# hinike/cairo

Measured on AMD Instinct MI355X. Metric: encoded Mpixels/s (p-frame, q=16) at 1/2/4/8 MI355X; bit-exact vs ref, higher is better.
Workload: dtype int16

## Files before the change

cairo_amd/__init__.py:

```python
from __future__ import annotations

import ctypes
import os
from dataclasses import dataclass

import numpy as np

_HERE = os.path.dirname(os.path.abspath(__file__))
LIB_PATH = os.path.join(_HERE, "_lib", "libcairo_amd.so")

BLOCK_DESC = np.dtype(
    [
        ("block_type", "<u4"),
        ("prediction_target", "u1"),
        ("pad", "u1"),
        ("motion_x", "<i2"),
        ("motion_y", "<i2"),
        ("sp_pred", "u1"),
        ("sp_amount", "u1"),
        ("sp_index", "u1"),
        ("q_index", "u1"),
        ("variance", "<i2"),
    ]
)
# ... 87 lines not shown
        "cairo_stream_payload_bits": (I, [P, I, ctypes.POINTER(ctypes.c_uint64)]),
        "cairo_bits_append": (I, [P, ctypes.c_uint64, ctypes.POINTER(ctypes.c_uint64), P, ctypes.c_uint64]),
        "evx_encoder_create": (I, [ctypes.POINTER(P)]),
        "evx_encoder_destroy": (I, [P]),
        "evx_encoder_clear": (I, [P]),
        "evx_encoder_insert_intra": (I, [P]),
        "evx_encoder_set_quality": (I, [P, ctypes.c_uint8]),
        "evx_encoder_encode": (I, [P, P, U, U, P]),
        "evx_encoder_set_ring": (I, [P, U]),
        "evx_encoder_peek": (I, [P, I, P]),
        "evx_encoder_set_device": (I, [P, I]),
        "evx_bitstream_create": (P, [U]),
        "evx_bitstream_destroy": (V, [P]),
        "evx_bitstream_data": (P, [P]),
        "evx_bitstream_occupancy": (U, [P]),
        "evx_bitstream_empty": (V, [P]),
        "evx_bitstream_write_bits": (I, [P, P, U]),
        "evx_decoder_create": (I, [ctypes.POINTER(P)]),
        "evx_decoder_destroy": (I, [P]),
        "evx_decoder_clear": (I, [P]),
        "evx_decoder_decode": (I, [P, P, P]),
        "evx_decoder_set_device": (I, [P, I]),
        "cairo_ctx_decode_frame": (I, [P, P, P, U, P]),
        "cairo_make_band4": (V, [P, U, U, U, U]),
        "cairo_version": (ctypes.c_char_p, []),
        "cairo_api_version": (I, []),
        "cairo_device_count": (I, []),
    }
    for name, (res, args) in sig.items():
        fn = getattr(L, name)
        fn.restype = res
        fn.argtypes = args
    if L.cairo_api_version() != API_VERSION:
        raise ImportError(f"{LIB_PATH} has C ABI version {L.cairo_api_version()}, these bindings expect "
                          f"{API_VERSION} (include/cairo_amd.h CAIRO_AMD_API_VERSION): rebuild with `make`")
    _lib = L
    return L


def _ck(status: int, what: str) -> None:
    if status != EVX_SUCCESS:
        raise CairoError(what, status)


def _ptr(a: np.ndarray) -> int:
    assert a.flags["C_CONTIGUOUS"]
    return a.ctypes.data


def _host_frame(rgb, width: int, height: int) -> int:
    if not isinstance(rgb, np.ndarray):
        raise TypeError("host frames are numpy arrays (pass on_device=True for a device address)")
    if rgb.dtype != np.uint8 or rgb.shape != (height, width, 3) or not rgb.flags["C_CONTIGUOUS"]:
        raise ValueError(f"frame must be a C-contiguous uint8 array of shape ({height}, {width}, 3), "
                         f"got {rgb.dtype} {rgb.shape}")
    return rgb.ctypes.data


def make_band4(w: int, h: int, t: int, seed: int = 1234) -> np.ndarray:
    out = np.empty((h, w, 3), np.uint8)
    lib().cairo_make_band4(_ptr(out), w, h, t, seed)
    return out


class _FrameResult(ctypes.Structure):
    _fields_ = [
        ("block_table", ctypes.c_void_p),
        ("coef_y", ctypes.c_void_p),
        ("coef_u", ctypes.c_void_p),
        ("coef_v", ctypes.c_void_p),
        ("wa", ctypes.c_uint32),
        ("ha", ctypes.c_uint32),
        ("wmb", ctypes.c_uint32),
        ("hmb", ctypes.c_uint32),
        ("index", ctypes.c_uint32),
        ("type", ctypes.c_uint32),
        ("quality", ctypes.c_uint32),
        ("feed", ctypes.c_void_p),
        ("feed_bits", ctypes.c_uint64),
        ("feed_status", ctypes.c_int32),
    ]


@dataclass
class FrameOutputs:

    table: np.ndarray
    coef_y: np.ndarray | None
    coef_u: np.ndarray | None
    coef_v: np.ndarray | None
    feed: np.ndarray | None = None
    feed_bits: int = 0
    feed_status: int = 0


def _view(addr: int, dtype, count: int) -> np.ndarray:
    buf = (ctypes.c_char * (count * np.dtype(dtype).itemsize)).from_address(addr)
    return np.frombuffer(buf, dtype=dtype, count=count)


class Context:

    def __init__(self, width: int, height: int, ring: int = 4, device: int = 0, stages: int = 96):
        self.L = lib()
        self.width, self.height, self.ring, self.device = width, height, ring, device
        self.wa, self.ha = (width + 15) & ~15, (height + 15) & ~15
        self.wmb, self.hmb = self.wa // 16, self.ha // 16
        p = ctypes.c_void_p()
        _ck(self.L.cairo_ctx_create_ex(width, height, ring, device, stages, ctypes.byref(p)), "cairo_ctx_create")
        self.h = p
        self._keep = {}

    def close(self) -> None:
        if self.h:
            self.L.cairo_ctx_destroy(self.h)
            self.h = None

    def __del__(self):
        try:
            self.close()
        except Exception:
            pass

    @property
    def stages(self) -> int:
        return int(self.L.cairo_ctx_stages(self.h))

    def submit(self, rgb, index: int, inter: bool, quality: int, on_device: bool = False) -> int:
        t = ctypes.c_int()
        ptr = rgb if on_device else _host_frame(rgb, self.width, self.height)
        _ck(
            self.L.cairo_ctx_submit(self.h, ptr, int(on_device), index, int(inter), quality, ctypes.byref(t)),
            "cairo_ctx_submit",
        )
        if not on_device:
            self._keep[t.value] = rgb
        return t.value

    def wait(self, ticket: int, copy: bool = True) -> FrameOutputs:
        r = _FrameResult()
        st = self.L.cairo_ctx_wait(self.h, ticket, ctypes.byref(r))
        if st != EVX_SUCCESS:
            raise CairoError("cairo_ctx_wait", st, self.timeout_info() if st == EVX_ERROR_HARDWAREFAIL else None)
        self._keep.pop(ticket, None)
        return self._outputs(r, copy)

    ACCT_FIELDS = ("coder_tasks", "coder_total", "coder_group_wait", "coder_window", "coder_search", "coder_inter",
                   "coder_dequeue", "coder_mbs", "helper_tasks", "helper_total", "helper_wait", "helper_deblock",
                   "helper_search", "helper_catchup", "helper_dequeue", "helper_chunks",
                   "win_bytes", "win_spec_unused_bytes", "zero_mv_bytes", "gran_poll_bytes", "rec_poll_bytes",
                   "win_stages", "searched_tasks", "inter_tasks", "coder_xform", "coder_publish", "coder_drain",
                   "coder_vm0", "coder_records", "coder_prebarrier", "coder_store_tail",
                   "search_eval", "search_barrier", "search_select", "subpel_eval", "subpel_barrier",
                   "subpel_select", "db_inputs", "db_filter", "db_write")

    def read_acct(self, reset: bool = False) -> dict:
        w = np.zeros(len(self.ACCT_FIELDS), np.uint64)
        _ck(self.L.cairo_ctx_read_acct(self.h, _ptr(w), len(w), int(reset)), "cairo_ctx_read_acct")
        return {k: int(w[i]) for i, k in enumerate(self.ACCT_FIELDS)}

    def timeout_info(self) -> dict | None:
        w = np.zeros(16, np.int32)
        _ck(self.L.cairo_ctx_timeout_info(self.h, _ptr(w), 16), "cairo_ctx_timeout_info")
        if not w[0]:
            return None
        d = {k: int(w[i]) for i, k in enumerate(TIMEOUT_FIELDS)}
        d["kind"] = WAIT_KINDS.get(d["kind"], str(d["kind"]))
        d["seen"] = (d.pop("seen_hi") & 0xFFFFFFFF) << 32 | (d.pop("seen_lo") & 0xFFFFFFFF)
        return d

    def _outputs(self, r, copy: bool) -> FrameOutputs:
        ny, nc = r.wa * r.ha, (r.wa // 2) * (r.ha // 2)
        mbs = r.wmb * r.hmb
        has_coef = bool(r.coef_y)
        feed = _view(r.feed, np.uint32, (r.feed_bits + 31) // 32) if r.feed_status == FEED_VALID else None
        out = FrameOutputs(
            _view(r.block_table, BLOCK_DESC, mbs),
            _view(r.coef_y, np.int16, ny).reshape(r.ha, r.wa) if has_coef else None,
            _view(r.coef_u, np.int16, nc).reshape(r.ha // 2, r.wa // 2) if has_coef else None,
            _view(r.coef_v, np.int16, nc).reshape(r.ha // 2, r.wa // 2) if has_coef else None,
            feed, int(r.feed_bits), int(r.feed_status),
        )
        if copy:
            cp = lambda a: None if a is None else a.copy()
            out = FrameOutputs(cp(out.table), cp(out.coef_y), cp(out.coef_u), cp(out.coef_v), cp(out.feed),
                               out.feed_bits, out.feed_status)
        return out

    def set_outputs(self, outputs: int) -> None:
        _ck(self.L.cairo_ctx_set_outputs(self.h, outputs), "cairo_ctx_set_outputs")

    def fetch_coef(self, ticket: int):
        r = _FrameResult()
        _ck(self.L.cairo_ctx_fetch_coef(self.h, ticket, ctypes.byref(r)), "cairo_ctx_fetch_coef")
        ny, nc = self.wa * self.ha, (self.wa // 2) * (self.ha // 2)
        return (_view(r.coef_y, np.int16, ny).reshape(self.ha, self.wa).copy(),
                _view(r.coef_u, np.int16, nc).reshape(self.ha // 2, self.wa // 2).copy(),
                _view(r.coef_v, np.int16, nc).reshape(self.ha // 2, self.wa // 2).copy())

    def release(self, ticket: int) -> None:
        _ck(self.L.cairo_ctx_release(self.h, ticket), "cairo_ctx_release")

    def encode_frame(self, rgb, index: int, inter: bool, quality: int, on_device: bool = False) -> FrameOutputs:
        t = self.submit(rgb, index, inter, quality, on_device)
        try:
            return self.wait(t, copy=True)
        finally:
            self.release(t)

    def sync(self) -> None:
        _ck(self.L.cairo_ctx_sync(self.h), "cairo_ctx_sync")

    def reset(self) -> None:
        _ck(self.L.cairo_ctx_reset(self.h), "cairo_ctx_reset")
        self._keep.clear()

    def read_planes(self, which: int):
        y = np.empty((self.ha, self.wa), np.int16)
        u = np.empty((self.ha // 2, self.wa // 2), np.int16)
        v = np.empty_like(u)
        _ck(self.L.cairo_ctx_read_planes(self.h, which, _ptr(y), _ptr(u), _ptr(v)), "read_planes")
        return y, u, v

    def read_inter(self):
        n = self.wmb * self.hmb * max(self.ring - 1, 0)
        d = np.zeros(n, BLOCK_DESC)
        s = np.zeros(n, np.int32)
        if n:
            _ck(self.L.cairo_ctx_read_inter(self.h, _ptr(d), _ptr(s)), "read_inter")
        return d, s

    def read_table(self):
        t = np.zeros(self.wmb * self.hmb, BLOCK_DESC)
        _ck(self.L.cairo_ctx_read_table(self.h, _ptr(t)), "read_table")
        return t

    def set_debug(self, flags: int) -> None:
        _ck(self.L.cairo_ctx_set_debug(self.h, flags), "set_debug")

    def read_predeblock(self):
        y = np.empty((self.ha, self.wa), np.int16)
        u = np.empty((self.ha // 2, self.wa // 2), np.int16)
        v = np.empty_like(u)
        _ck(self.L.cairo_ctx_read_predeblock(self.h, _ptr(y), _ptr(u), _ptr(v)), "read_predeblock")
        return y, u, v

    def read_stamps(self):
        n_mb, n_db = self.hmb * self.wmb * 12, self.hmb * 256
        fw = n_mb + n_db
        ng = (self.wmb + 3) // 4
        n_it = MAX_BATCH * self.hmb * ng * 12
        out = np.zeros(MAX_BATCH * fw + 2 + n_it, np.uint64)
        _ck(self.L.cairo_ctx_read_stamps(self.h, _ptr(out)), "read_stamps")
        fr = out[: MAX_BATCH * fw].reshape(MAX_BATCH, fw)
        return (fr[:, :n_mb].reshape(MAX_BATCH, self.hmb, self.wmb, 12), fr[:, n_mb:].reshape(MAX_BATCH, self.hmb, 256),
                out[MAX_BATCH * fw:MAX_BATCH * fw + 2], out[MAX_BATCH * fw + 2:].reshape(MAX_BATCH, self.hmb, ng, 12))

    def set_profiling(self, enable: bool) -> None:
        _ck(self.L.cairo_ctx_set_profiling(self.h, int(enable)), "set_profiling")

    def take_timings(self):
        ms = (ctypes.c_double * 4)()
        n = ctypes.c_int()
        _ck(self.L.cairo_ctx_take_timings(self.h, ms, ctypes.byref(n)), "take_timings")
        return list(ms), n.value

    def busy_intervals(self) -> np.ndarray:
        n = ctypes.c_int()
        _ck(self.L.cairo_ctx_busy_intervals(self.h, None, 0, ctypes.byref(n)), "busy_intervals")
        out = np.zeros((max(n.value, 1), 2), np.float64)
        _ck(self.L.cairo_ctx_busy_intervals(self.h, _ptr(out), n.value, ctypes.byref(n)), "busy_intervals")
        return out[: n.value]

    def set_batch(self, frames: int) -> None:
        _ck(self.L.cairo_ctx_set_batch(self.h, frames), "set_batch")

    def set_workgroups(self, rows: int = 0) -> None:
        _ck(self.L.cairo_ctx_set_workgroups(self.h, rows), "set_workgroups")

    def set_helpers(self, helpers: int = 0) -> None:
        _ck(self.L.cairo_ctx_set_helpers(self.h, helpers), "set_helpers")

    def max_workgroups(self) -> int:
        return int(self.L.cairo_ctx_max_workgroups(self.h))

    def flush(self) -> None:
        _ck(self.L.cairo_ctx_flush(self.h), "cairo_ctx_flush")

    def peer_info(self, cross_device: bool = False) -> bytes:
        rec = (ctypes.c_uint8 * PEER_SIZE)()
        _ck(self.L.cairo_ctx_peer_info(self.h, int(cross_device), rec), "cairo_ctx_peer_info")
        return bytes(rec)

    def join_group(self, rank: int, peers: list) -> None:
        buf = b"".join(peers)
        assert len(buf) == PEER_SIZE * len(peers)
        arr = (ctypes.c_uint8 * len(buf)).from_buffer_copy(buf)
        _ck(self.L.cairo_ctx_join_group(self.h, len(peers), rank, arr), "cairo_ctx_join_group")


MIRROR_SLOTS = 16


def group_layout(n: int, size: int, ring: int, stages: int, mirror: bool = False) -> dict:
    slots = -(-ring // size)
    t = n // size
    slot = (n % size) * slots + t % slots if mirror else t % slots
# ... 323 lines not shown
```

cairo_amd/csrc/kernels.h:

```cpp
#pragma once

#include <hip/hip_runtime.h>
#include <stdint.h>

#include "evx_defs.h"

namespace cairo {

struct PlaneSet {
  int16_t* y;
  int16_t* u;
  int16_t* v;
};

__host__ __device__ inline PlaneSet ring_slot(int16_t* base, size_t slot_elems, int wa, int ha,
                                              int k) {
  PlaneSet p;
  p.y = base + (size_t)k * slot_elems;
  p.u = p.y + (size_t)wa * ha;
  p.v = p.u + (size_t)(wa / 2) * (ha / 2);
  return p;
}

constexpr int kGranulesPerMB = 192;
constexpr int kGranuleStride = 193;

__host__ __device__ inline uint32_t pack_inter_desc(const BlockDesc& d) {
  return (d.block_type & 7u) | ((uint32_t)(d.prediction_target & 3) << 3) | ((uint32_t)(d.sp_pred & 1) << 5) |
         ((uint32_t)(d.sp_amount & 1) << 6) | ((uint32_t)(d.sp_index & 15) << 7) |
         (((uint32_t)d.motion_x & 0x7Fu) << 11) | (((uint32_t)d.motion_y & 0x7Fu) << 18);
}
__host__ __device__ inline BlockDesc unpack_inter_desc(uint32_t w) {
  BlockDesc d;
  d.block_type = w & 7u;
  d.prediction_target = (uint8_t)((w >> 3) & 3);
  d.pad = 0;
  d.sp_pred = (uint8_t)((w >> 5) & 1);
  d.sp_amount = (uint8_t)((w >> 6) & 1);
  d.sp_index = (uint8_t)((w >> 7) & 15);
  d.motion_x = (int16_t)((int32_t)(w << 14) >> 25);
  d.motion_y = (int16_t)((int32_t)(w << 7) >> 25);
  d.q_index = 0;
  d.variance = 0;
  return d;
}

constexpr int kStampPhases = 12;
constexpr int kDbStamps = 256;
constexpr int kIStamps = 12;
__host__ __device__ inline size_t stamp_frame_words(int wmb, int hmb) {
  return (size_t)wmb * hmb * kStampPhases + (size_t)hmb * kDbStamps;
}

struct TimeoutInfo {
  static constexpr int kKind = 0;
  static constexpr int kEpoch = 1;
  static constexpr int kIndex = 2;
  static constexpr int kRow = 3;
  static constexpr int kMember = 4;
  static constexpr int kNeed = 5;
  static constexpr int kOn = 6;
  static constexpr int kSeenLo = 7;
  static constexpr int kSeenHi = 8;
  static constexpr int kClaim = 9;
  static constexpr int kWords = 16;
};
enum TimeoutKind : int32_t {
  kWaitRecords = 1,
  kWaitGranule = 2,
  kWaitPrevProgress = 3,
  kWaitRowAbove = 4,
  kWaitBatch = 5,
  kWaitInjected = 6,
  kWaitHostMark = 9,
};

#ifndef CAIRO_ACCT
#define CAIRO_ACCT 0
#endif
constexpr int kAcctShards = 64, kAcctWords = 40;
struct Acct {
  static constexpr int kCoderTasks = 0, kCoderTotal = 1, kCoderGroupWait = 2, kCoderWindow = 3, kCoderSearch = 4,
                       kCoderInter = 5, kCoderDequeue = 6, kCoderMBs = 7;
  static constexpr int kHelperTasks = 8, kHelperTotal = 9, kHelperWait = 10, kHelperDeblock = 11, kHelperSearch = 12,
                       kHelperCatchup = 13, kHelperDequeue = 14, kHelperChunks = 15;
  static constexpr int kWinBytes = 16, kWinSpecUnused = 17, kZeroMvBytes = 18, kGranPollBytes = 19,
                       kRecPollBytes = 20, kWinStages = 21, kSearchedTasks = 22, kInterTasks = 23;
  static constexpr int kCoderXform = 24, kCoderPublish = 25, kCoderDrain = 26;
  static constexpr int kCoderVm0 = 27, kCoderRecords = 28, kCoderPreBarrier = 29;
  static constexpr int kCoderStoreTail = 30;
  static constexpr int kSrchEval = 31, kSrchBarrier = 32, kSrchSelect = 33, kSubEval = 34, kSubBarrier = 35,
                       kSubSelect = 36;
  static constexpr int kDbInputs = 37, kDbFilter = 38, kDbWrite = 39;
};

#ifndef CAIRO_MAX_BATCH
#define CAIRO_MAX_BATCH 48
#endif
constexpr int kMaxBatch = CAIRO_MAX_BATCH;
constexpr int kMaxGroup = 16;
constexpr int kMaxPush = kMaxRing;

struct FrameDesc {
  const uint8_t* rgb;
  const uint8_t* host_rgb;
  int index;
  int inter;
  int quality;
  uint32_t epoch;
  int slot;
  int decode;
  PlaneSet recon[kMaxRing];
  PlaneSet stale;
  PlaneSet coef;
  PlaneSet push[kMaxPush];
  int npush;
  PlaneSet coef_prev;
  uint64_t* progress;
  const uint64_t* prev_progress;
  const uint64_t* prev2_progress;
  int sys;
  int member;
  const BlockDesc* host_table;
  const int16_t* host_coef;
};

struct FrameArgs {
  int wa, ha;
  int w, h;
  int wmb, hmb;
  int ring;
  int index, inter, quality;
  int decode;
  uint32_t epoch;
  PlaneSet in;
  PlaneSet coef;
  PlaneSet coef_prev;
  PlaneSet recon[kMaxRing];
  PlaneSet stale;
  PlaneSet push[kMaxPush];
  int npush;
  BlockDesc* table;
  BlockDesc* inter_desc;
  void* reserved0;
  uint64_t* granules;
  int32_t* err;
  int32_t* sticky;
  int member;
  int inject;
  int ng;
  int nref;
  int32_t* inter_done;
  uint64_t* progress;
  const uint64_t* prev_progress;
  const uint64_t* prev2_progress;
  int sys;
  int db_shift;
  uint64_t* stamps;
  uint64_t* acct;
  uint64_t* istamps;
  const uint8_t* rgb;
};

struct EngineArgs;
FrameArgs make_frame_view(const EngineArgs& e, const FrameDesc& f, int j);

struct SyncLayout {
  static constexpr int kErr = 0;
  static constexpr int kDone = 4;
  static constexpr int kLabelOff = 5;
  static constexpr int kTicketRows = 8;
  static constexpr int kTicketHelpers = 16;
  static constexpr int kFlags = 24;
  __host__ __device__ static int frame_words(int hmb, int ng) { return hmb * ng; }
  __host__ __device__ static int inter_done(int hmb, int ng, int j) { return kFlags + frame_words(hmb, ng) * j; }
  __host__ __device__ static int words(int hmb, int ng) { return kFlags + frame_words(hmb, ng) * kMaxBatch + 8; }
};

struct EngineArgs {
  int wa, ha, w, h, wmb, hmb, ring;
  int nframes;
  const FrameArgs* fa;
  int16_t* src_base;
  size_t plane_elems;
  BlockDesc* table_base;
  BlockDesc* idesc_base;
  void* reserved0;
  uint64_t* gran_base;
  int32_t* sync;
  int32_t* sticky;
  int inject;
  uint64_t* stamps;
  uint64_t* acct;
  int n_helpers, n_rows;
  int32_t* trace;
  const int32_t* order[2];
  const int32_t* seg[2];
  int nlab[2];
  int decode;
  const FrameArgs* pfa;
  const int32_t* porder[2];
  const int32_t* pseg[2];
  int32_t* psync;
  int ptotal;
  int slope;
};

constexpr int kOrderSlope = 5;

constexpr int kPrioFrameMBs = 4000;

constexpr int kLabels = 8;
constexpr int kBandMinRows = 100;
constexpr int kBandPools = 3;
__host__ __device__ inline int task_label(int frame, int row, int hmb) {
  (void)frame;
  return row * kLabels / hmb;
}

struct ConvertArgs {
  int w, h, wa, nframes;
  const uint8_t* rgb[kMaxBatch];
  PlaneSet in[kMaxBatch];
  const uint4* fa_host;
  uint4* fa_dev;
  int fa_chunks;
  int32_t* sync;
  int sync_words;
};
hipError_t launch_convert_batch(const ConvertArgs& c, hipStream_t s);
hipError_t launch_engine(const EngineArgs& e, hipStream_t s);
hipError_t launch_batch_wait(int32_t* sync, int tasks, int32_t* sticky, hipStream_t s);
hipError_t engine_blocks_per_cu(int* n);
hipError_t launch_unpack_granules(const EngineArgs& e, int j, PlaneSet dst, hipStream_t s);

hipError_t launch_yuv_to_rgb(PlaneSet src, int wa, int w, int h, uint8_t* rgb, hipStream_t s);

hipError_t launch_kat_transform(const int16_t* src, const int16_t* pred, int16_t* coef,
                                int16_t* recon, const uint8_t* qtype, int32_t* qvar,
                                int count, hipStream_t s);

}
```

cairo_amd/csrc/kernels.hip:

```cpp
#include "kernels.h"

namespace cairo {

typedef const __attribute__((address_space(4))) FrameArgs FA;
#define RECON_AT(a, k)                                                                   \
  ((k) == 1 ? planes((a).recon[1]) : (k) == 2 ? planes((a).recon[2]) : (k) == 3 ? planes((a).recon[3]) \
                                                                              : planes((a).recon[0]))
__host__ __device__ inline PlaneSet planes(const __attribute__((address_space(4))) PlaneSet& p) {
  PlaneSet r;
  r.y = p.y;
  r.u = p.u;
  r.v = p.v;
  return r;
}


__constant__ int16_t kLut8[64] = {
    128, 128,  128,  128,  128,  128,  128,  128,
    126, 106,  71,   25,   -25,  -71,  -106, -126,
    118, 49,   -49,  -118, -118, -49,  49,   118,
    106, -25,  -126, -71,  71,   126,  25,   -106,
    91,  -91,  -91,  91,   91,   -91,  -91,  91,
    71,  -126, 25,   106,  -106, -25,  126,  -71,
    49,  -118, 118,  -49,  -49,  118,  -118, 49,
// ... 399 lines not shown
  const int16_t* py = &p.y[(size_t)(y + (l >> 2)) * wa + x + (l & 3) * 4];
  int cw = wa >> 1;
  Px6 r;
  r.y0 = py[0];
  r.y1 = py[1];
  r.y2 = py[2];
  r.y3 = py[3];
  r.u = p.u[(size_t)((y >> 1) + (l >> 3)) * cw + (x >> 1) + (l & 7)];
  r.v = p.v[(size_t)((y >> 1) + (l >> 3)) * cw + (x >> 1) + (l & 7)];
  return r;
}

__device__ __forceinline__ int lerp_px(int a, int b, int quarter) {
  return quarter ? (int16_t)(round_out(3 * a + b, 2) / 4) : (int16_t)(round_out(a + b, 1) / 2);
}
__device__ __forceinline__ uint32_t lerp_half_bb(uint32_t a, uint32_t b) {
  const uint32_t t = a + b;
  return (t + ((t >> 16) & 1)) >> 1;
}
__device__ __forceinline__ uint32_t lerp_quarter_bb3(uint32_t a3, uint32_t b) {
  const uint32_t t = a3 + b;
  return (t + 1 + ((t >> 17) & 1)) >> 2;
}
__device__ __forceinline__ uint32_t lerp_quarter_bb(uint32_t a, uint32_t b) { return lerp_quarter_bb3(3 * a, b); }
__device__ __forceinline__ uint32_t absdiff_b(uint32_t x, uint32_t y) {
  return __builtin_amdgcn_sad_u16(x, y, 0);
}

__device__ __forceinline__ void inter_cand_row(const Window& w, int wx, int wy, int i, const SrcRow& s, int thr,
                                               int& sad, int& mad) {
  const int sh = (wx & 1) * 2;
  const uint32_t* row = (const uint32_t*)&w.y[(wy + i) * kWinLP] + (wx >> 1);
  uint32_t d[9];
#pragma unroll
  for (int k = 0; k < 9; k++) d[k] = row[k];
  uint32_t sm = 0;
#pragma unroll
  for (int k = 0; k < 8; k++) sm = __builtin_amdgcn_sad_u16(s.y[k], __builtin_amdgcn_alignbyte(d[k + 1], d[k], sh), sm);
  sad = row16_sum((int)sm);
  mad = kMadFar;
  if (__ballot(mad_needed(sad, thr))) {
    u16x2 m1 = {0, 0}, m2 = {0, 0};
    uint32_t dummy = 0;
#pragma unroll
    for (int k = 0; k < 8; k++) pk_diff(s.y[k], __builtin_amdgcn_alignbyte(d[k + 1], d[k], sh), dummy, m1, m2);
    const int cr = (wy >> 1) + (i >> 1), cc = (wx >> 1) + (i & 1) * 4, shc = (cc & 1) * 2;
    const uint32_t* ru = (const uint32_t*)&w.u[cr * kWinCP] + (cc >> 1);
    const uint32_t* rv = (const uint32_t*)&w.v[cr * kWinCP] + (cc >> 1);
    const uint32_t u0 = ru[0], u1 = ru[1], u2 = ru[2], v0 = rv[0], v1 = rv[1], v2 = rv[2];
    pk_diff(s.u[0], __builtin_amdgcn_alignbyte(u1, u0, shc), dummy, m1, m2);
    pk_diff(s.u[1], __builtin_amdgcn_alignbyte(u2, u1, shc), dummy, m1, m2);
    pk_diff(s.v[0], __builtin_amdgcn_alignbyte(v1, v0, shc), dummy, m1, m2);
    pk_diff(s.v[1], __builtin_amdgcn_alignbyte(v2, v1, shc), dummy, m1, m2);
    const u16x2 m = __builtin_elementwise_max(m1, m2);
    mad = row16_max(max((int)m.x, (int)m.y));
  }
}

__device__ __forceinline__ SrcRow load_src_rows(const PlaneSet& in, int wa, int px, int py, int i) {
  SrcRow s;
  const uint4* ry = (const uint4*)(in.y + (size_t)(py + i) * wa + px);
  const uint4 r0 = ry[0], r1 = ry[1];
  s.y[0] = r0.x, s.y[1] = r0.y, s.y[2] = r0.z, s.y[3] = r0.w;
  s.y[4] = r1.x, s.y[5] = r1.y, s.y[6] = r1.z, s.y[7] = r1.w;
  const size_t co = (size_t)((py >> 1) + (i >> 1)) * (wa >> 1) + (px >> 1) + (i & 1) * 4;
  const uint2 u2 = *(const uint2*)(in.u + co), v2 = *(const uint2*)(in.v + co);
  s.u[0] = u2.x, s.u[1] = u2.y, s.v[0] = v2.x, s.v[1] = v2.y;
#pragma unroll
  for (int k = 0; k < 8; k++) s.y[k] ^= 0x80008000u;
#pragma unroll
  for (int k = 0; k < 2; k++) s.u[k] ^= 0x80008000u, s.v[k] ^= 0x80008000u;
  return s;
}

__device__ __forceinline__ void sad_mad(const Px6& s, const Px6& c, int& sad, int& mad) {
  int d0 = abs(s.y0 - c.y0), d1 = abs(s.y1 - c.y1), d2 = abs(s.y2 - c.y2), d3 = abs(s.y3 - c.y3);
  int du = abs(s.u - c.u), dv = abs(s.v - c.v);
  sad = wave_sum(d0 + d1 + d2 + d3);
  mad = wave_max(max(max(max(d0, d1), max(d2, d3)), max(du, dv)));
}

struct Sel {
  int bx, by, sad, mad, ssd, sp_idx, sp_amt, sp_en;
};

__device__ __forceinline__ void accept_int(Sel& s, int cx, int cy, int sad, int mad, int px, int py,
                                           int thr) {
  int ssd = (cx - px) * (cx - px) + (cy - py) * (cy - py);
  bool acc = (s.mad < thr) ? (mad < s.mad || (mad == s.mad && ssd < s.ssd))
                           : (sad < s.sad || (sad == s.sad && ssd < s.ssd && sad < kSadGate) ||
                              mad < thr);
  if (acc) {
    s.bx = cx;
    s.by = cy;
    s.sad = sad;
    s.ssd = ssd;
    s.mad = mad;
  }
}
__device__ __forceinline__ void accept_sub(Sel& s, int idx, int quarter, int sad, int mad,
                                           int thr) {
  bool acc = (s.mad < thr) ? (mad < s.mad) : ((sad < s.sad && sad < kSadGate) || mad < thr);
  if (acc) {
    s.sp_en = 1;
    s.sp_amt = quarter;
    s.sp_idx = idx;
    s.sad = sad;
    s.mad = mad;
  }
}



__device__ __forceinline__ uint32_t row0_min(uint32_t v) {
  v = min(v, (uint32_t)__builtin_amdgcn_mov_dpp((int)v, 0x128, 0xF, 0xF, false));
  v = min(v, (uint32_t)__builtin_amdgcn_mov_dpp((int)v, 0x124, 0xF, 0xF, false));
  v = min(v, (uint32_t)__builtin_amdgcn_mov_dpp((int)v, 0x122, 0xF, 0xF, false));
  v = min(v, (uint32_t)__builtin_amdgcn_mov_dpp((int)v, 0x121, 0xF, 0xF, false));
  return (uint32_t)__builtin_amdgcn_readlane((int)v, 0);
}

__device__ __forceinline__ uint32_t key_copy(int mad, int ssd, int idx) {
  return ((uint32_t)min(mad, 65535) << 16) | ((uint32_t)min(ssd, 4095) << 4) | (uint32_t)idx;
}
__device__ __forceinline__ uint32_t key_sad(int sad, int ssd, int idx) {
  if (sad < kSadGate)
    return ((uint32_t)sad << 18) | ((uint32_t)min(ssd, 16383) << 4) | (uint32_t)idx;
  return 0x80000000u | ((uint32_t)min(sad, (1 << 27) - 1) << 4) | (uint32_t)idx;
}

__device__ __forceinline__ void select_int(Sel& s, bool valid, int cx, int cy, int sad, int mad,
                                           int px, int py, int thr, int lane) {
  const int c = lane & 15;
  const bool live = lane < 16 && valid;
  const int ssd = (cx - px) * (cx - px) + (cy - py) * (cy - py);
  const uint32_t fm = (uint32_t)__ballot(live && mad < thr);
  int w = -1;
  if (s.mad < thr || fm) {
    const int f = s.mad < thr ? -1 : (int)__builtin_ctz(fm);
    const uint32_t k = row0_min(live && c >= f ? key_copy(mad, ssd, c + 1) : 0xFFFFFFFFu);
    if (f >= 0) w = (int)(k & 15) - 1;
    else if (k < key_copy(s.mad, s.ssd, 0)) w = (int)(k & 15) - 1;
  } else {
    const uint32_t k = row0_min(live ? key_sad(sad, ssd, c + 1) : 0xFFFFFFFFu);
    if (k < key_sad(s.sad, s.ssd, 0)) w = (int)(k & 15) - 1;
  }
  if (w >= 0) {
    s.bx = __builtin_amdgcn_readlane(cx, w);
    s.by = __builtin_amdgcn_readlane(cy, w);
    s.sad = __builtin_amdgcn_readlane(sad, w);
    s.ssd = __builtin_amdgcn_readlane(ssd, w);
    s.mad = __builtin_amdgcn_readlane(mad, w);
  }
}

__device__ __forceinline__ void select_sub(Sel& s, bool valid, int sad, int mad, int thr, int lane) {
  const int c = lane & 15;
  const bool live = lane < 16 && valid;
  const uint32_t fm = (uint32_t)__ballot(live && mad < thr);
  int w = -1;
  if (s.mad < thr || fm) {
    const int f = s.mad < thr ? -1 : (int)__builtin_ctz(fm);
    const uint32_t k = row0_min(live && c >= f ? (((uint32_t)min(mad, 65535) << 5) | (uint32_t)(c + 1))
                                               : 0xFFFFFFFFu);
    if (f >= 0) w = (int)(k & 31) - 1;
    else if (k < ((uint32_t)min(s.mad, 65535) << 5)) w = (int)(k & 31) - 1;
  } else {
    const uint32_t k =
        row0_min(live && sad < kSadGate ? (((uint32_t)sad << 5) | (uint32_t)(c + 1)) : 0xFFFFFFFFu);
    if (k < ((uint32_t)min(s.sad, 1 << 26) << 5)) w = (int)(k & 31) - 1;
  }
  if (w >= 0) {
    const int n = w >> 1, k9 = n < 4 ? n : n + 1;
    s.sp_en = 1;
    s.sp_amt = w & 1;
    s.sp_idx = frac_index(k9 % 3 - 1, k9 / 3 - 1);
    s.sad = __builtin_amdgcn_readlane(sad, w);
    s.mad = __builtin_amdgcn_readlane(mad, w);
  }
}

__device__ __forceinline__ bool in_frame(int x, int y, int wa, int ha) {
  return x >= 0 && x <= wa - kMB && y >= 0 && y <= ha - kMB;
}

__device__ __forceinline__ BlockDesc make_desc(const Sel& s, int px, int py, int thr, bool intra,
                                               int target) {
  BlockDesc d;
  uint32_t t = intra ? kIntra : 0u;
  if (s.bx != px || s.by != py || s.sp_en) t |= kMotion;
  if (s.mad < thr) t |= kCopy;
  d.block_type = t;
  d.prediction_target = (uint8_t)target;
  d.pad = 0;
  d.motion_x = (int16_t)(s.bx - px);
  d.motion_y = (int16_t)(s.by - py);
  d.sp_pred = (uint8_t)s.sp_en;
  d.sp_amount = (uint8_t)s.sp_amt;
  d.sp_index = (uint8_t)s.sp_idx;
  d.q_index = 0;
  d.variance = 0;
  return d;
}


constexpr int kLvl1Rows = 77, kLvl1Cols = 112;

__device__ __forceinline__ int wg_broadcast(volatile int* slot, int v) {
  if (threadIdx.x == 0) *slot = v;
  __syncthreads();
  const int r = *slot;
  __syncthreads();
  return r;
}

struct DbLds;
struct DbState;
__device__ __forceinline__ bool deblock_chunk_ready(FA& a, int r, const DbState& st);
__device__ __forceinline__ void deblock_chunk(FA& a, int r, DbLds& D, DbState& st, bool known_ready = false);
__device__ __forceinline__ bool deblock_pending(FA& a, const DbState& st);

template <bool kDeblock = true>
__device__ __forceinline__ void helper_wait(FA& a, int back, int r, int rr, int need, DbLds& D, DbState& st,
                                            int* flag) {
  volatile int* vflag = flag;
  const uint64_t* pp = back == 1 ? a.prev_progress : a.prev2_progress;
  uint64_t t0 = 0;
  const uint64_t ta = acct_now();
  uint64_t tdb = 0;
  for (;;) {
    int d = 0;
    if (threadIdx.x == 0) {
      const uint64_t pv = pp ? progress_peer(a.sys, pp + rr) : ~0ull;
      const bool dbr = kDeblock && deblock_pending(a, st) && deblock_chunk_ready(a, r, st);
      if (a.inject && r == min(1, a.hmb - 1)) {
        report_timeout(a, kWaitInjected, r, need, rr | (back << 16), pv);
        d = 1;
      } else if (pv >= tagged(a.epoch - back, need)) {
        d = 1;
      } else if (dbr) {
        d = 2;
      } else {
        const uint64_t now = __builtin_amdgcn_s_memrealtime();
        if (!t0) t0 = now;
        __builtin_amdgcn_s_sleep(1);
        if (__hip_atomic_load(a.err, __ATOMIC_RELAXED, __HIP_MEMORY_SCOPE_AGENT)) {
          d = 1;
        } else if (now - t0 > 200000000ull) {
          report_timeout(a, kWaitPrevProgress, r, need, rr | (back << 16), pv);
          d = 1;
        }
      }
    }
    d = wg_broadcast(vflag, d);
    if (d == 1) break;
    if (kDeblock && d == 2) {
      const uint64_t tb = acct_now();
      deblock_chunk(a, r, D, st, true);
      tdb += acct_now() - tb;
    }
  }
  if (threadIdx.x == 0) {
    acquire_fence(a.sys);
    asm volatile("s_waitcnt vmcnt(0)" ::: "memory");
  }
  __syncthreads();
  acct_add(a.acct, Acct::kHelperWait, acct_now() - ta - tdb);
}

struct InterLds {
  Window win;
  int need[4];
  int full;
  int lvl2[6][4];
  alignas(16) int16_t src[4][384];
  int zsad[kMaxRing][4], zmad[kMaxRing][4];
};

__device__ __forceinline__ void group_source(FA& a, int r, int g, InterLds& L) {
  const int wave = threadIdx.x >> 6, lane = threadIdx.x & 63, x = 4 * g + wave;
  if (x >= a.wmb || lane >= 48) return;
  const PlaneSet in = planes(a.in);
  const int px = x * kMB, py = r * kMB;
  const int16_t* gsrc;
  if (lane < 32) {
    gsrc = in.y + (size_t)(py + (lane >> 1)) * a.wa + px + 8 * (lane & 1);
  } else {
    const int k = lane - 32;
    gsrc = pick(in, 1 + (k >> 3)) + (size_t)((py >> 1) + (k & 7)) * (a.wa >> 1) + (px >> 1);
  }
  *(uint4*)&L.src[wave][8 * lane] = *(const uint4*)gsrc;
}

__device__ __forceinline__ void src_dma(FA& a, int x, int r, int16_t* dst) {
  const int lane = threadIdx.x;
  if (lane >= 48) return;
  const PlaneSet in = planes(a.in);
  const int px = x * kMB, py = r * kMB;
  const int16_t* gsrc = lane < 32 ? in.y + (size_t)(py + (lane >> 1)) * a.wa + px + 8 * (lane & 1)
                                  : pick(in, 1 + ((lane - 32) >> 3)) +
                                        (size_t)((py >> 1) + (lane & 7)) * (a.wa >> 1) + (px >> 1);
  __builtin_amdgcn_global_load_lds((const void*)gsrc, (lds_void*)dst, 16, 0, 0);
}

__device__ __forceinline__ Px6 src_px_lds(const InterLds& L, int wave) {
  const int l = threadIdx.x & 63;
// ... 837 lines not shown
      asm volatile("s_waitcnt vmcnt(0)" ::: "memory");
      __syncthreads();
    }
    for (int bx = 0; bx < a0.wmb; bx++) {
      FA* ap = opaque_view(&a0);
      const int px = bx * kMB, mb = by * ap->wmb + bx;
      trace(tr, 1, bx);
      trace(tr, 2, (int)ap->epoch * 1000 + by);
      stamp(*ap, mb, 0);
      if (ap->stamps && tid == 0) ap->stamps[(size_t)mb * kStampPhases + 10] = __builtin_amdgcn_s_memtime();
      if (!kDecode && bx + 1 < ap->wmb) src_dma(*ap, bx + 1, by, L.src[(bx + 1) & 1]);
      const bool fresh_col = by > 0 && bx != 0 && bx + 2 < ap->wmb && tid < kGranulesPerMB;
      const uint64_t* fresh_gp = fresh_col ? gran_at(*ap, bx + 2, by - 1, tid) : nullptr;
      const uint64_t fresh_g = fresh_col ? gran_ld(fresh_gp) : 0;
      const bool gstart = (bx & 3) == 0;
      const bool early = !kDecode && gstart;
      const int nref = ap->inter ? ap->ring - 1 : 0;
      uint64_t rg[kMaxRing - 1][2];
      auto issue_records = [&]() {
#pragma unroll
        for (int o = 0; o < kMaxRing - 1; o++) {
          if (o >= nref) break;
          const uint64_t* r = (const uint64_t*)&ap->inter_desc[o * mbs + mb];
          rg[o][0] = gran_ld(r);
          rg[o][1] = gran_ld(r + 1);
        }
      };
      if (!early) issue_records();
#ifdef CAIRO_ACCT_STORE_TAIL
      {
        const uint64_t ts = acct_now();
        asm volatile("s_waitcnt vmcnt(0)" ::: "memory");
        acct_add(ap->acct, Acct::kCoderStoreTail, acct_now() - ts);
      }
#endif
      uint64_t tacc = acct_now();
      const bool by_tag = ap->inter;
      const uint64_t* grec = (const uint64_t*)&ap->inter_desc[mb];
      uint64_t rd0 = 0;
      if (early && tid == 0)
        rd0 = by_tag ? gran_ld(grec)
                     : (uint64_t)__hip_atomic_load(&ap->inter_done[by * ap->ng + (bx >> 2)], __ATOMIC_RELAXED,
                                                   __HIP_MEMORY_SCOPE_AGENT);
      bool ready0 = false;
      if (gstart && !early) {
        if (tid == 0) {
          if (by_tag) rec_settle(*ap, grec, gran_ld(grec), by, mb);
          else wait_records(*ap, by, bx >> 2);
        }
        acquire_after_wait(ap->sys);
        acct_add(ap->acct, Acct::kCoderGroupWait, acct_now() - tacc);
      }
      tacc = acct_now();

      if (by > 0) {
        if (bx == 0) {
          int lx[9], ly[9], n = 0;
          for (int r = max(by - 3, 0); r <= by - 1; r++)
            for (int c = 0; c <= 2 && c < ap->wmb; c++) lx[n] = c, ly[n++] = r;
          for (int k = tid; k < n * kGranulesPerMB; k += 256) {
            const int i = k / kGranulesPerMB, kk = k - i * kGranulesPerMB;
            const uint64_t* gp = gran_at(*ap, lx[i], ly[i], kk);
            win_put_k(L.win, oy, lx[i], ly[i], kk, gran_settle(*ap, gp, gran_ld(gp), by));
          }
        } else if (fresh_col) {
          win_put_k(L.win, oy, bx + 2, by - 1, tid,
                    gran_settle(*ap, fresh_gp, fresh_g, by));
        }
      }
      acct_add(ap->acct, Acct::kCoderWindow, acct_now() - tacc);
      const uint64_t tv0 = acct_now();
      if (!kDecode) __builtin_amdgcn_s_waitcnt(kWaitVm0);
      acct_add(ap->acct, Acct::kCoderVm0, acct_now() - tv0);
      if (early && tid == 0) {
        ready0 = by_tag ? (uint32_t)(rd0 >> 32) == ap->epoch : (int)rd0 >= ap->nref;
        if (ready0) acquire_fence(ap->sys);
      }
      SrcRow s;
      if (!kDecode) {
        const uint32_t* m = (const uint32_t*)L.src[bx & 1];
#pragma unroll
        for (int k = 0; k < 8; k++) s.y[k] = m[gi * 8 + k] ^ 0x80008000u;
        const int co = (gi >> 1) * 4 + (gi & 1) * 2;
        s.u[0] = m[128 + co] ^ 0x80008000u, s.u[1] = m[128 + co + 1] ^ 0x80008000u;
        s.v[0] = m[160 + co] ^ 0x80008000u, s.v[1] = m[160 + co + 1] ^ 0x80008000u;
      }
      const bool pf3 = by >= 3 && bx + 3 < ap->wmb, pf2 = by >= 2 && bx + 3 < ap->wmb;
      const bool pfs = by + 1 < ap->hmb && bx + 1 < ap->wmb;
      uint64_t pg3 = 0, pg2 = 0;
      uint32_t pst = 0;
      if (tid < kGranulesPerMB) {
        if (pf3) pg3 = gran_ld(gran_at(*ap, bx + 3, by - 3, tid));
        if (pf2) pg2 = gran_ld(gran_at(*ap, bx + 3, by - 2, tid));
        if (pfs && !early) pst = *(const uint32_t*)win_src(cs, ap->wa, bx, by + 1, tid);
      }

      BlockDesc ib;
      int ib_sad = 0;
      int ipa[2] = {0, 0}, ipb[2] = {0, 0};
      auto load_inter = [&]() {
#pragma unroll
        for (int o = 0; o < kMaxRing - 1; o++) {
          if (o >= nref) break;
          const uint64_t* r = (const uint64_t*)&ap->inter_desc[o * mbs + mb];
          const BlockDesc rd = unpack_inter_desc((uint32_t)uni((int)rec_settle(*ap, r, rg[o][0], by, mb)));
          const int rs = uni((int)rec_settle(*ap, r + 1, rg[o][1], by, mb));
          if (o == 0) {
            ib = rd, ib_sad = rs;
          } else {
            const bool ci = (rd.block_type & kCopy) != 0, cb = (ib.block_type & kCopy) != 0;
            if (ci != cb ? ci : rs < ib_sad) ib = rd, ib_sad = rs;
          }
        }
        if (nref == 0) return;
        const BlockDesc& d = ib;
        const PlaneSet rp = RECON_AT(*ap, d.prediction_target);
        const bool mot = (d.block_type & kMotion) != 0, sp = mot && d.sp_pred;
        const int mx = px + (mot ? d.motion_x : 0), my = py + (mot ? d.motion_y : 0);
        int dx = 0, dy = 0;
        if (sp) frac_dir(d.sp_index, &dx, &dy);
        _Pragma("unroll") for (int bi = 0; bi < 2; bi++) if (bi < nblk) {
          ipa[bi] = pred_at(rp, ap->wa, (wave + 4 * bi) * 64 + lane, mx, my);
          if (sp) ipb[bi] = pred_at(rp, ap->wa, (wave + 4 * bi) * 64 + lane, mx + dx, my + dy);
        }
      };
      const uint64_t tr0 = acct_now();
      if (!early) load_inter();
      stamp(*ap, mb, 1);
      const uint64_t tr1 = acct_now();
      __syncthreads();
      stamp(*ap, mb, 2);
      tacc = acct_now();
      acct_add(ap->acct, Acct::kCoderRecords, tr1 - tr0);
      acct_add(ap->acct, Acct::kCoderPreBarrier, tacc - tr1);

      BlockDesc d;
      bool from_inter = false;
      int wpv[2] = {0, 0};
      if (!kDecode) {
        Sel sel;
        {
          int sm = 0;
  #pragma unroll
          for (int k = 0; k < 16; k++) sm += abs(src_px(s.y, k));
          sel.sad = uni(row16_sum(sm));
        }
        sel.bx = px;
        sel.by = py;
        sel.mad = INT32_MAX;
        sel.ssd = INT32_MAX;
        sel.sp_idx = sel.sp_amt = sel.sp_en = 0;
        int buf = 0;
        uint64_t t_ev = 0, t_ba = 0, t_se = 0;
  #pragma unroll 1
        for (int stage = 0; stage < ((CAIRO_ATTR_SKIP & 16) ? 0 : 5); stage++) {
          const int step = stage == 0 ? kRadius : (kRadius >> stage);
          const int jlo = stage == 0 ? -2 * kRadius : -step;
          const int bx0 = sel.bx, by0 = sel.by;
          const uint64_t ts0 = acct_now();
          if (grp < 9) {
            const int c = min(grp, 8);
            const int cx = bx0 - step + (c % 3) * step, cy = by0 + jlo + (c / 3) * step;
            const bool ok = intra_valid(cx, cy, px, py, ap->wa, ap->ha);
            int sad, mad;
            cand_row(L.win, oy, cx, ok ? cy : py - 48, gi, s, thr, sad, mad);
            if (gi == 0 && grp < 9) {
              L.cand[buf][grp][0] = ok ? sad : -1;
              L.cand[buf][grp][1] = mad;
            }
          }
          const uint64_t ts1 = acct_now();
          __syncthreads();
          const uint64_t ts2 = acct_now();
          {
            const int c = lane & 15;
            const int vs = L.cand[buf][c][0], vm = L.cand[buf][c][1];
            const int cx = bx0 - step + (c % 3) * step, cy = by0 + jlo + (c / 3) * step;
            select_int(sel, c < 9 && vs >= 0, cx, cy, vs, vm, px, py, thr, lane);
          }
          buf ^= 1;
          if (CAIRO_ACCT) {
            const uint64_t ts3 = uni((int)sel.bx) == -99999 ? 0 : acct_now();
            t_ev += ts1 - ts0, t_ba += ts2 - ts1, t_se += ts3 - ts2;
          }
        }
        acct_add(ap->acct, Acct::kSrchEval, t_ev);
        acct_add(ap->acct, Acct::kSrchBarrier, t_ba);
        acct_add(ap->acct, Acct::kSrchSelect, t_se);
        stamp(*ap, mb, 3);
        if (!(CAIRO_ATTR_SKIP & 16)) {
          const int bx0 = sel.bx, by0 = sel.by;
          const int q = (grp >> 2) & 1, nn = (grp & 3) | ((grp >> 3) << 2), c = 2 * nn + q;
          const int k9 = nn < 4 ? nn : nn + 1;
          const int tx = bx0 + k9 % 3 - 1, ty = by0 + k9 / 3 - 1;
          const bool ok = intra_valid(tx, ty, px, py, ap->wa, ap->ha);
          int sad, mad;
          const uint64_t ts0 = acct_now();
          subpel_row(L.win, oy, bx0, ok ? by0 : py - 48, tx, ok ? ty : py - 48, uni(q), gi, s, thr, sad, mad);
          if (gi == 0) {
            L.cand[buf][c][0] = ok ? sad : -1;
            L.cand[buf][c][1] = mad;
          }
          const uint64_t ts1 = acct_now();
          __syncthreads();
          const uint64_t ts2 = acct_now();
          const int vs = L.cand[buf][lane & 15][0], vm = L.cand[buf][lane & 15][1];
          sel.sp_idx = sel.sp_amt = sel.sp_en = 0;
          select_sub(sel, vs >= 0, vs, vm, thr, lane);
          if (CAIRO_ACCT) {
            const uint64_t ts3 = uni((int)sel.sp_idx) == -99999 ? 0 : acct_now();
            acct_add(ap->acct, Acct::kSubEval, ts1 - ts0);
            acct_add(ap->acct, Acct::kSubBarrier, ts2 - ts1);
            acct_add(ap->acct, Acct::kSubSelect, ts3 - ts2);
          }
        }
        stamp(*ap, mb, 4);
        acct_add(ap->acct, Acct::kCoderSearch, acct_now() - tacc);
        if (early) {
          tacc = acct_now();
          if (tid == 0) {
            if (!ready0) {
              if (by_tag) rec_settle(*ap, grec, gran_ld(grec), by, mb);
              else wait_records(*ap, by, bx >> 2);
              acquire_fence(ap->sys);
            }
            asm volatile("s_waitcnt vmcnt(0)" ::: "memory");
          }
          __syncthreads();
          acct_add(ap->acct, Acct::kCoderGroupWait, acct_now() - tacc);
          tacc = acct_now();
          if (tid < kGranulesPerMB && pfs) pst = *(const uint32_t*)win_src(cs, ap->wa, bx, by + 1, tid);
          issue_records();
          load_inter();
          acct_add(ap->acct, Acct::kCoderInter, acct_now() - tacc);
        }
        d = make_desc(sel, px, py, thr, true, 0);
        int best_sad = sel.sad;

        if (nref > 0) {
          const bool ci = (ib.block_type & kCopy) != 0, cb = (d.block_type & kCopy) != 0;
          if (ci != cb ? ci : ib_sad < best_sad) {
            d = ib;
            best_sad = ib_sad;
            from_inter = true;
            const bool sp = (d.block_type & kMotion) && d.sp_pred;
            _Pragma("unroll") for (int bi = 0; bi < 2; bi++) {
              asm volatile("" : "+v"(ipa[bi]), "+v"(ipb[bi]));
              wpv[bi] = sp ? lerp_px(ipa[bi], ipb[bi], d.sp_amount) : ipa[bi];
            }
          }
        }
      } else {
        const uint4 tw = *(const uint4*)&ap->table[mb];
        d = uni_desc_words(tw);
        d.q_index = (uint8_t)(uni((int)tw.w) >> 8);
        if (!(d.block_type & kIntra)) {
          from_inter = true;
          const PlaneSet rp = RECON_AT(*ap, d.prediction_target);
          const bool mot = (d.block_type & kMotion) != 0, sp = mot && d.sp_pred;
          int dx = 0, dy = 0;
          if (sp) frac_dir(d.sp_index, &dx, &dy);
          _Pragma("unroll") for (int bi = 0; bi < 2; bi++) if (bi < nblk)
            wpv[bi] = pred_global(rp, ap->wa, (wave + 4 * bi) * 64 + lane, px + (mot ? d.motion_x : 0),
                                  py + (mot ? d.motion_y : 0), sp, dx, dy, d.sp_amount);
        }
      }
      ap = opaque_view(ap);
      stamp(*ap, mb, 5);
      const uint64_t tx5 = acct_now();
      int svp[2] = {0, 0};
      if (!kDecode) {
        _Pragma("unroll") for (int bi = 0; bi < 2; bi++) if (bi < nblk) {
          int pl, ex, ey;
          elem_coords((wave + 4 * bi) * 64 + lane, 0, 0, pl, ex, ey);
          svp[bi] = L.src[bx & 1][pl == 0 ? ey * 16 + ex : 256 + (pl - 1) * 64 + ey * 8 + ex];
        }
      }

      const uint32_t type = d.block_type;
      const bool has_pred = type != kIntra;
      const bool intra_path = (type & kIntra) && !(type & kMotion);
      int pv[2] = {0, 0}, cf[2] = {0, 0};
      if (from_inter) {
        pv[0] = wpv[0];
        pv[1] = wpv[1];
      } else if (has_pred) {
        const int mx = px + d.motion_x, my = py + d.motion_y;
        const bool sp = d.sp_pred;
        int dx = 0, dy = 0;
        if (sp) frac_dir(d.sp_index, &dx, &dy);
        _Pragma("unroll") for (int bi = 0; bi < 2; bi++) if (bi < nblk) {
          const int e = (wave + 4 * bi) * 64 + lane;
          int pl, ex, ey;
          elem_coords(e, mx, my, pl, ex, ey);
          int v = win_px(L.win, oy, pl, ex, ey);
          if (sp) {
            int nx, ny;
            elem_coords(e, mx + dx, my + dy, pl, nx, ny);
            v = lerp_px(v, win_px(L.win, oy, pl, nx, ny), d.sp_amount);
          }
          pv[bi] = v;
        }
      }
      if (!(type & kCopy) && !kDecode) {
        _Pragma("unroll") for (int bi = 0; bi < 2; bi++) if (bi < nblk) {
          const int b = wave + 4 * bi, e = b * 64 + lane;
          int pl, ex, ey;
          elem_coords(e, px, py, pl, ex, ey);
          const int sv = svp[bi];
          const int16_t res = has_pred ? (int16_t)(sv - pv[bi]) : (int16_t)sv;
          cf[bi] = (CAIRO_ATTR_SKIP & 64) ? res
                   : (__ballot(res != 0) ? fdct_lane(&L.bufA[b * 64], &L.bufB[b * 64], lane, res) : 0);
        }
      }
      stamp(*ap, mb, 6);
      if (tid < kGranulesPerMB) {
        if (pf3)
          win_put_k(L.win, oy, bx + 3, by - 3, tid,
                    gran_settle(*ap, gran_at(*ap, bx + 3, by - 3, tid), pg3, by));
        if (pf2)
          win_put_k(L.win, oy, bx + 3, by - 2, tid,
                    gran_settle(*ap, gran_at(*ap, bx + 3, by - 2, tid), pg2, by));
        if (pfs) win_put_k(L.win, oy, bx, by + 1, tid, pst);
      }
      if (!(type & kCopy)) {
        int qp;
        if (!kDecode) {
          int32_t v2;
          qp = vaq_mb(L.red, wave, lane, cf[0], ap->quality, &v2);
          d.q_index = (uint8_t)qp;
          d.variance = (int16_t)v2;
        } else {
          qp = d.q_index;
        }
        _Pragma("unroll") for (int bi = 0; bi < 2; bi++) if (bi < nblk) {
          const int b = wave + 4 * bi, e = b * 64 + lane;
          int16_t qv;
          if (!kDecode) {
            qv = (CAIRO_ATTR_SKIP & 64) ? (int16_t)cf[bi] : quant_elem(e, cf[bi], qp, intra_path);
            coef_store_pair(*ap, e, px, py, qv);
          } else {
// ... 478 lines not shown
```

Measured before the change: 7022.

## Speculatively evaluate next search stage alongside current stage to skip passes

The integer motion search now uses the otherwise idle groups 8-15 to evaluate the next, half-step stage around the current centre in the same pass. A new two-row selector first checks the current-stage candidates. If the centre stays put, it takes the result of the speculative stage and advances two stages, saving a barrier and a select round. This costs extra SAD work on every speculative stage and makes the selection logic more complex, and the result must stay bit-exact with the sequential search. Accounting counters for pass counts are added.

Result: faster. 7151, median of 6 (+1.8%).

```diff
diff --git a/cairo_amd/__init__.py b/cairo_amd/__init__.py
--- a/cairo_amd/__init__.py
+++ b/cairo_amd/__init__.py
@@ -263,7 +263,8 @@
                    "win_stages", "searched_tasks", "inter_tasks", "coder_xform", "coder_publish", "coder_drain",
                    "coder_vm0", "coder_records", "coder_prebarrier", "coder_store_tail",
                    "search_eval", "search_barrier", "search_select", "subpel_eval", "subpel_barrier",
-                   "subpel_select", "db_inputs", "db_filter", "db_write")
+                   "subpel_select", "db_inputs", "db_filter", "db_write",
+                   "search_passes", "search_mbs_2pass", "search_mbs_3pass", "search_mbs_4pass")
 
     def read_acct(self, reset: bool = False) -> dict:
         w = np.zeros(len(self.ACCT_FIELDS), np.uint64)
diff --git a/cairo_amd/csrc/kernels.h b/cairo_amd/csrc/kernels.h
--- a/cairo_amd/csrc/kernels.h
+++ b/cairo_amd/csrc/kernels.h
@@ -78,7 +78,7 @@
 #ifndef CAIRO_ACCT
 #define CAIRO_ACCT 0
 #endif
-constexpr int kAcctShards = 64, kAcctWords = 40;
+constexpr int kAcctShards = 64, kAcctWords = 44;
 struct Acct {
   static constexpr int kCoderTasks = 0, kCoderTotal = 1, kCoderGroupWait = 2, kCoderWindow = 3, kCoderSearch = 4,
                        kCoderInter = 5, kCoderDequeue = 6, kCoderMBs = 7;
@@ -92,6 +92,7 @@
   static constexpr int kSrchEval = 31, kSrchBarrier = 32, kSrchSelect = 33, kSubEval = 34, kSubBarrier = 35,
                        kSubSelect = 36;
   static constexpr int kDbInputs = 37, kDbFilter = 38, kDbWrite = 39;
+  static constexpr int kSrchPasses = 40, kSrchPasses2 = 41, kSrchPasses3 = 42, kSrchPasses4 = 43;
 };
 
 #ifndef CAIRO_MAX_BATCH
diff --git a/cairo_amd/csrc/kernels.hip b/cairo_amd/csrc/kernels.hip
--- a/cairo_amd/csrc/kernels.hip
+++ b/cairo_amd/csrc/kernels.hip
@@ -575,6 +575,44 @@
     s.ssd = __builtin_amdgcn_readlane(ssd, w);
     s.mad = __builtin_amdgcn_readlane(mad, w);
   }
+}
+
+__device__ __forceinline__ bool select_int2(Sel& s, bool two, bool valid, int cx, int cy, int sad, int mad,
+                                            int px, int py, int thr, int lane) {
+  const int c = lane & 15;
+  const bool live = lane < (two ? 32 : 16) && valid;
+  const int ssd = (cx - px) * (cx - px) + (cy - py) * (cy - py);
+  const uint32_t fm2 = (uint32_t)__ballot(live && mad < thr);
+  const uint32_t fm0 = fm2 & 0xFFFFu, fm1 = fm2 >> 16;
+  const bool copy = s.mad < thr;
+  const uint32_t fmr = lane < 16 ? fm0 : fm1;
+  const int f = copy || !fmr ? -1 : (int)__builtin_ctz(fmr);
+  uint32_t key = 0xFFFFFFFFu;
+  if (live) key = copy || fmr ? (c >= f ? key_copy(mad, ssd, c + 1) : 0xFFFFFFFFu) : key_sad(sad, ssd, c + 1);
+  key = min(key, (uint32_t)__builtin_amdgcn_mov_dpp((int)key, 0x128, 0xF, 0xF, false));
+  key = min(key, (uint32_t)__builtin_amdgcn_mov_dpp((int)key, 0x124, 0xF, 0xF, false));
+  key = min(key, (uint32_t)__builtin_amdgcn_mov_dpp((int)key, 0x122, 0xF, 0xF, false));
+  key = min(key, (uint32_t)__builtin_amdgcn_mov_dpp((int)key, 0x121, 0xF, 0xF, false));
+  const uint32_t kc = key_copy(s.mad, s.ssd, 0), ks = key_sad(s.sad, s.ssd, 0);
+  auto winner = [&](uint32_t k, uint32_t fm) -> int {
+    if (!copy && fm) return (int)(k & 15) - 1;
+    return k < (copy ? kc : ks) ? (int)(k & 15) - 1 : -1;
+  };
+  int w = winner((uint32_t)__builtin_amdgcn_readlane((int)key, 0), fm0);
+  bool second = false;
+  if (two && w < 0) {
+    second = true;
+    w = winner((uint32_t)__builtin_amdgcn_readlane((int)key, 16), fm1);
+    if (w >= 0) w += 16;
+  }
+  if (w >= 0) {
+    s.bx = __builtin_amdgcn_readlane(cx, w);
+    s.by = __builtin_amdgcn_readlane(cy, w);
+    s.sad = __builtin_amdgcn_readlane(sad, w);
+    s.ssd = __builtin_amdgcn_readlane(ssd, w);
+    s.mad = __builtin_amdgcn_readlane(mad, w);
+  }
+  return second;
 }
 
 __device__ __forceinline__ void select_sub(Sel& s, bool valid, int sad, int mad, int thr, int lane) {
@@ -1718,21 +1756,29 @@
         sel.sp_idx = sel.sp_amt = sel.sp_en = 0;
         int buf = 0;
         uint64_t t_ev = 0, t_ba = 0, t_se = 0;
+        int passes = 0;
   #pragma unroll 1
-        for (int stage = 0; stage < ((CAIRO_ATTR_SKIP & 16) ? 0 : 5); stage++) {
+        for (int stage = 0; stage < ((CAIRO_ATTR_SKIP & 16) ? 0 : 5);) {
           const int step = stage == 0 ? kRadius : (kRadius >> stage);
           const int jlo = stage == 0 ? -2 * kRadius : -step;
+          const int n0 = stage == 0 ? 9 : 8;
+          const bool spec = stage >= 1 && stage < 4;
           const int bx0 = sel.bx, by0 = sel.by;
           const uint64_t ts0 = acct_now();
-          if (grp < 9) {
-            const int c = min(grp, 8);
-            const int cx = bx0 - step + (c % 3) * step, cy = by0 + jlo + (c / 3) * step;
-            const bool ok = intra_valid(cx, cy, px, py, ap->wa, ap->ha);
-            int sad, mad;
-            cand_row(L.win, oy, cx, ok ? cy : py - 48, gi, s, thr, sad, mad);
-            if (gi == 0 && grp < 9) {
-              L.cand[buf][grp][0] = ok ? sad : -1;
-              L.cand[buf][grp][1] = mad;
+          {
+            const bool second = stage >= 1 && grp >= 8;
+            const int c = second ? grp - 8 : grp;
+            const int k9 = stage == 0 || c < 4 ? c : c + 1;
+            const int st = second ? step >> 1 : step;
+            if (second ? spec : grp < n0) {
+              const int cx = bx0 - st + (k9 % 3) * st, cy = by0 + (second ? -st : jlo) + (k9 / 3) * st;
+              const bool ok = intra_valid(cx, cy, px, py, ap->wa, ap->ha);
+              int sad, mad;
+              cand_row(L.win, oy, cx, ok ? cy : py - 48, gi, s, thr, sad, mad);
+              if (gi == 0) {
+                L.cand[buf][grp][0] = ok ? sad : -1;
+                L.cand[buf][grp][1] = mad;
+              }
             }
           }
           const uint64_t ts1 = acct_now();
@@ -1740,19 +1786,28 @@
           const uint64_t ts2 = acct_now();
           {
             const int c = lane & 15;
-            const int vs = L.cand[buf][c][0], vm = L.cand[buf][c][1];
-            const int cx = bx0 - step + (c % 3) * step, cy = by0 + jlo + (c / 3) * step;
-            select_int(sel, c < 9 && vs >= 0, cx, cy, vs, vm, px, py, thr, lane);
+            const bool row1 = (lane & 16) != 0;
+            const int e = row1 ? 8 + (c & 7) : c;
+            const int vs = L.cand[buf][e][0], vm = L.cand[buf][e][1];
+            const int k9 = stage == 0 || c < 4 ? c : c + 1;
+            const int st = row1 ? step >> 1 : step;
+            const int cx = bx0 - st + (k9 % 3) * st, cy = by0 + (row1 ? -st : jlo) + (k9 / 3) * st;
+            stage += select_int2(sel, spec, c < (row1 ? 8 : n0) && vs >= 0, cx, cy, vs, vm, px, py, thr, lane) ? 2 : 1;
           }
           buf ^= 1;
           if (CAIRO_ACCT) {
             const uint64_t ts3 = uni((int)sel.bx) == -99999 ? 0 : acct_now();
             t_ev += ts1 - ts0, t_ba += ts2 - ts1, t_se += ts3 - ts2;
+            passes++;
           }
         }
         acct_add(ap->acct, Acct::kSrchEval, t_ev);
         acct_add(ap->acct, Acct::kSrchBarrier, t_ba);
         acct_add(ap->acct, Acct::kSrchSelect, t_se);
+        if (CAIRO_ACCT && passes >= 3) {
+          acct_add(ap->acct, Acct::kSrchPasses, (uint64_t)passes);
+          acct_add(ap->acct, Acct::kSrchPasses2 + (passes - 3), 1);
+        }
         stamp(*ap, mb, 3);
         if (!(CAIRO_ATTR_SKIP & 16)) {
           const int bx0 = sel.bx, by0 = sel.by;
```
